# yukara-ikemiya/friendly-stable-audio-tools

Hardware: AMD Instinct MI355X
Metric: audio-seconds/sec @44.1kHz stereo, 100-step DPM++, SA-Open-1.0 shape (higher is better)
Workload: dtype fp16; 1 GPU; Stable-Audio-Open-1.0 DiT shape (24 layers, D=1536, S=1025, CFG 7 -> 2 sequences/prompt) + Oobleck decode, 1 prompt(s)/GPU x 47.55 s, 100 DPM-Solver++(3M) SDE steps; prompts_per_gpu=1, codec_dtype=fp16, sampler_steps=100, layernorm=fused, cross_attention=fused, sample_size=2097152, parallelism=dp1 (rank-strided prompts, one all-gather)

## Files before the change

### friendly-stable-audio-tools_amd/csrc/gemm_bf16.hip

```cpp
#include <stdlib.h>

#include <type_traits>

#include "attn_core.h"
#include <algorithm>

#include "sat_common.h"

namespace {

template <int EPI, int MI, int NI, bool LNC = false, bool QKN = false>
__device__ __forceinline__ void gemm_epilogue(const GemmArgs& g, f32x16 (&acc)[MI][NI], const int mw, const int nw, const int half,
                                              const int l31, const float2* ln = nullptr, const float* lc1 = nullptr,
                                              const float* lc2 = nullptr) {
    const int M = g.M, N = g.N;
    (void)N;

    if constexpr (EPI == EPI_F32) {
        float* __restrict__ C = g.C;
        const int ldc = g.ldc;
        float bia[NI];
#pragma unroll
        for (int j = 0; j < NI; ++j) bia[j] = g.bias ? g.bias[nw + j * 32 + l31] : 0.f;
        const bool accum = g.accumulate != 0;
// ... 344 lines not shown
            const int m = mw + i * 32 + l31;
            const int mc = m < M ? m : M - 1;
            const int b = mc / S;
            const int s = mc - b * S;
            const int ob = (kind & 4) ? ((b * S) & 3) : 0;
            if constexpr (LNC) {
                const float2 st = ln[i * 32 + l31];
#pragma unroll
                for (int j = 0; j < 2; ++j)
#pragma unroll
                    for (int q = 0; q < 4; ++q) {
                        const f32x4 c1 = *reinterpret_cast<const f32x4*>(lc1 + j * 32 + q * 8 + 4 * half);
                        const f32x4 c2 = *reinterpret_cast<const f32x4*>(lc2 + j * 32 + q * 8 + 4 * half);
#pragma unroll
                        for (int e = 0; e < 4; ++e) acc[i][j][4 * q + e] = st.y * (acc[i][j][4 * q + e] - st.x * c1[e]) + c2[e];
                    }
            }
            if constexpr (QKN) {
                if (kind & 16) {
                    float ss = 0.f;
#pragma unroll
                    for (int j = 0; j < 2; ++j)
#pragma unroll
                        for (int r = 0; r < 16; ++r) ss += acc[i][j][r] * acc[i][j][r];
                    unsigned a = __float_as_uint(ss), b = a;
                    half_swap(a, b);
                    const float inv = rsqrtf(fmaxf(__uint_as_float(a) + __uint_as_float(b), 1e-24f));
#pragma unroll
                    for (int j = 0; j < 2; ++j)
#pragma unroll
                        for (int r = 0; r < 16; ++r) acc[i][j][r] *= inv;
                }
            }
            if (kind & 2) {
                if constexpr (!ROPE_PRE) {
                    rcs[i][0] = *reinterpret_cast<const f32x4*>(he.rope_cos + (size_t)s * 16 + 4 * half);
                    rcs[i][1] = *reinterpret_cast<const f32x4*>(he.rope_cos + (size_t)s * 16 + 8 + 4 * half);
                    rsn[i][0] = *reinterpret_cast<const f32x4*>(he.rope_sin + (size_t)s * 16 + 4 * half);
                    rsn[i][1] = *reinterpret_cast<const f32x4*>(he.rope_sin + (size_t)s * 16 + 8 + 4 * half);
                }
                const f32x4 cs0 = rcs[i][0], cs1 = rcs[i][1], sn0 = rsn[i][0], sn1 = rsn[i][1];
#pragma unroll
                for (int r = 0; r < 8; ++r) {
                    const float cs = (r < 4) ? cs0[r & 3] : cs1[r & 3];
                    const float sn = (r < 4) ? sn0[r & 3] : sn1[r & 3];
                    const float x1 = acc[i][0][r], x2 = acc[i][0][r + 8];
                    acc[i][0][r] = x1 * cs - x2 * sn;
                    acc[i][0][r + 8] = x2 * cs + x1 * sn;
                }
            }
            if (kind & 8) {
#pragma unroll
                for (int j = 0; j < 2; ++j)
#pragma unroll
                    for (int r = 0; r < 16; ++r) acc[i][j][r] *= he.qscale;
            }
            op_t* row = dst + ((size_t)(b * he.heads + head) * Spad + s + ob) * 64 + 8 * half;
#pragma unroll
            for (int j = 0; j < 2; ++j) {
                unsigned pk[8];
#pragma unroll
                for (int q = 0; q < 4; ++q) {
                    pk[2 * q] = pack_op2(acc[i][j][4 * q], acc[i][j][4 * q + 1]);
                    pk[2 * q + 1] = pack_op2(acc[i][j][4 * q + 2], acc[i][j][4 * q + 3]);
                }
                half_swap(pk[0], pk[2]);
                half_swap(pk[1], pk[3]);
                half_swap(pk[4], pk[6]);
                half_swap(pk[5], pk[7]);
                if (qfrag) {
#pragma unroll
                    for (int e = 0; e < 8; ++e) qfrag[j][e] = pk[e];
                    continue;
                }
                if (m < M) {
                    *reinterpret_cast<u32x4*>(row + j * 32) = u32x4{pk[0], pk[1], pk[2], pk[3]};
                    *reinterpret_cast<u32x4*>(row + j * 32 + 16) = u32x4{pk[4], pk[5], pk[6], pk[7]};
                }
            }
        }
    }
}

template <int MI, bool PRE = false>
__device__ __forceinline__ void gemm_epilogue_f32_staged(const GemmArgs& g, f32x16 (&acc)[MI][2], float* ep, const int mw, const int nw,
                                                         const int lane, const f32x4* pre = nullptr) {
    const int half = lane >> 5, l31 = lane & 31;
    const int M = g.M;
    const int prow = lane >> 4;
    const int c4 = (lane & 15) * 4;
    const bool accum = g.accumulate != 0;
    const f32x4 bia = g.bias ? *reinterpret_cast<const f32x4*>(g.bias + nw + c4) : f32x4{0.f, 0.f, 0.f, 0.f};
#pragma unroll
    for (int i = 0; i < MI; ++i) {
#pragma unroll
        for (int j = 0; j < 2; ++j)
#pragma unroll
            for (int r = 0; r < 16; ++r) ep[((r & 3) + 8 * (r >> 2) + 4 * half) * 64 + j * 32 + l31] = acc[i][j][r];
#pragma unroll
        for (int grp = 0; grp < 2; ++grp) {
            f32x4 old[4];
#pragma unroll
            for (int p4 = 0; p4 < 4; ++p4) {
                const int m = mw + i * 32 + (grp * 4 + p4) * 4 + prow;
                if constexpr (PRE) old[p4] = pre[grp * 4 + p4];
                else old[p4] = (accum && m < M) ? *reinterpret_cast<const f32x4*>(g.C + (size_t)m * g.ldc + nw + c4) : f32x4{0.f, 0.f, 0.f, 0.f};
            }
#pragma unroll
            for (int p4 = 0; p4 < 4; ++p4) {
                const int row = (grp * 4 + p4) * 4 + prow;
                const int m = mw + i * 32 + row;
                f32x4 v = *reinterpret_cast<const f32x4*>(ep + row * 64 + c4) + bia;
                if (m < M && g.gate) v *= *reinterpret_cast<const f32x4*>(g.gate + (size_t)(m / g.gate_rows) * g.gate_ld + nw + c4);
                v += old[p4];
                if (m < M) *reinterpret_cast<f32x4*>(g.C + (size_t)m * g.ldc + nw + c4) = v;
                if (g.xb) {
                    opx4 xr;
                    float sum = 0.f, sq = 0.f;
#pragma unroll
                    for (int e = 0; e < 4; ++e) {
                        xr[e] = f32_to_op(v[e]);
                        const float f = op_to_f32(xr[e]);
                        sum += f;
                        sq += f * f;
                    }
                    sum = row16_sum(sum);
                    sq = row16_sum(sq);
                    if (m < M) {
                        *reinterpret_cast<opx4*>(g.xb + (size_t)m * g.N + nw + c4) = xr;
                        if ((lane & 15) == 0)
                            *reinterpret_cast<float2*>(g.ln_part_out + ((size_t)m * (g.N >> 6) + (nw >> 6)) * 2) = make_float2(sum, sq);
                    }
                }
            }
        }
    }
}

template <int BM, int BN, int WM, int WN, int EPIX>
__global__ __launch_bounds__(WM * WN * 64) void gemm_kernel(GemmArgs g) {
    sat_f16_saturate();
    constexpr int EPI = EPIX == EPI_HEADS_QKN ? EPI_HEADS : EPIX == EPI_ACT16 ? EPI_SWIGLU : EPIX;
    constexpr bool QKN = EPIX == EPI_HEADS_QKN || EPIX == EPI_ACT16;
    constexpr int NT = WM * WN * 64;
    constexpr int TM = BM / WM;
    constexpr int TN = BN / WN;
    static_assert(TN == 64, "wave tile is TM x 64");
    constexpr int MI = TM / 32;
    constexpr int NI = 2;
    constexpr int A_CH = BM * 8 / NT;
    constexpr int B_CH = BN * 8 / NT;
    static_assert(A_CH >= 1 && B_CH >= 1, "tile too small for the block");
    constexpr int STAGE_BYTES = (BM + BN) * 128;

    extern __shared__ __attribute__((aligned(16))) char smem[];

    const int tid = threadIdx.x;
    const int lane = tid & 63;
    const int wave = tid >> 6;
    const int wm = wave / WN;
    const int wn = wave % WN;
    const int half = lane >> 5;
    const int l31 = lane & 31;

    const int M = g.M, N = g.N, K = g.K;
    const int tiles_m = (M + BM - 1) / BM;
    const int tiles_n = N / BN;
    const int bid = xcd_remap(blockIdx.x, gridDim.x);
    int tm, tn;
    if (tiles_m <= tiles_n) {
        tn = bid / tiles_m;
        tm = bid - tn * tiles_m;
    } else {
        tm = bid / tiles_n;
        tn = bid - tm * tiles_n;
    }
    const int m0 = tm * BM;
    const int n0 = tn * BN;

    const op_t* __restrict__ A = g.A;
    const op_t* __restrict__ W = g.W;
// ... 110 lines not shown
    int tm, tn;
    if (tiles_m <= tiles_n) {
        tn = bid / tiles_m;
        tm = bid - tn * tiles_m;
    } else {
        tm = bid / tiles_n;
        tn = bid - tm * tiles_n;
    }
    const int m0 = tm * BM;
    const int n0 = tn * BN;

    const op_t* a_ptr[A_CH];
#pragma unroll
    for (int i = 0; i < A_CH; ++i) {
        int q = i * NT + tid;
        int row = q >> 3, pos = q & 7;
        int c = pos ^ ((row >> 1) & 7);
        int gm = m0 + row;
        gm = gm < M ? gm : M - 1;
        a_ptr[i] = g.A + (size_t)gm * K + c * 8;
    }
    const op_t* b_ptr[B_CH];
#pragma unroll
    for (int i = 0; i < B_CH; ++i) {
        int q = i * NT + tid;
        int row = q >> 3, pos = q & 7;
        int c = pos ^ ((row >> 1) & 7);
        b_ptr[i] = g.W + (size_t)(n0 + row) * K + c * 8;
    }

    f32x16 acc[MI][NI];
#pragma unroll
    for (int i = 0; i < MI; ++i)
#pragma unroll
        for (int j = 0; j < NI; ++j)
#pragma unroll
            for (int r = 0; r < 16; ++r) acc[i][j][r] = 0.f;

    auto stage_in = [&](int kt, int stage) {
        char* sa = smem + stage * STAGE_BYTES;
        char* sb = sa + BM * 128;
#pragma unroll
        for (int i = 0; i < A_CH; ++i)
            __builtin_amdgcn_global_load_lds((const __attribute__((address_space(1))) void*)(a_ptr[i] + kt * 64),
                                             (__attribute__((address_space(3))) void*)(sa + (i * NT + wave * 64) * 16), 16, 0, 0);
#pragma unroll
        for (int i = 0; i < B_CH; ++i)
            __builtin_amdgcn_global_load_lds((const __attribute__((address_space(1))) void*)(b_ptr[i] + kt * 64),
                                             (__attribute__((address_space(3))) void*)(sb + (i * NT + wave * 64) * 16), 16, 0, 0);
    };
    auto compute = [&](int stage) {
        const char* sa = smem + stage * STAGE_BYTES;
        const char* sb = sa + BM * 128;
#pragma unroll
        for (int ks = 0; ks < 4; ++ks) {
            opx8 af[MI], bfr[NI];
#pragma unroll
            for (int i = 0; i < MI; ++i)
                af[i] = *reinterpret_cast<const opx8*>(sa + lds_tile_off(wm * TM + i * 32 + l31, ks * 2 + half));
#pragma unroll
            for (int j = 0; j < NI; ++j)
                bfr[j] = *reinterpret_cast<const opx8*>(sb + lds_tile_off(wn * TN + j * 32 + l31, ks * 2 + half));
#pragma unroll
            for (int i = 0; i < MI; ++i)
#pragma unroll
                for (int j = 0; j < NI; ++j)
                    acc[i][j] = mfma_32x32x16(af[i], bfr[j], acc[i][j]);
        }
    };

    const int nk = K / 64;
    stage_in(0, 0);
    __syncthreads();
    for (int kt = 0; kt < nk - 1; ++kt) {
        stage_in(kt + 1, (kt + 1) & 1);
        compute(kt & 1);
        __syncthreads();
    }
    compute((nk - 1) & 1);

    gemm_epilogue<EPI, MI, NI, false, QKN>(g, acc, m0 + wm * TM, n0 + wn * TN, half, l31);
}

template <int BK>
__device__ __forceinline__ int lds_off_bk(int row, int chunk) {
    if constexpr (BK == 128) return row * 256 + ((chunk ^ (row & 15)) << 4);
    else if constexpr (BK == 64) return row * 128 + ((chunk ^ ((row >> 1) & 7)) << 4);
    else return row * 64 + ((chunk ^ ((row >> 2) & 3)) << 4);
}

template <int BM, int BN, int BK, int WM, int WN, int NS, int EPIX, int FP8 = 0, int KG = 1, bool DIL = false>
__global__ __launch_bounds__(KG * WM * WN * 64) void gemm_pipe_kernel(GemmArgs g) {
    sat_f16_saturate();
    constexpr int EPI = EPIX == EPI_HEADS_QKN ? EPI_HEADS : EPIX == EPI_ACT16 ? EPI_SWIGLU : EPIX;
    constexpr bool QKN = EPIX == EPI_HEADS_QKN || EPIX == EPI_ACT16;
    static_assert(!QKN || FP8 == 0, "qk_norm / plain activation: 16-bit operands only");
    static_assert(KG == 1 || (KG == 2 && EPI == EPI_F32 && FP8 == 0 && BK == 64 && BM / WM == 64 && BN / WN == 64),
                  "K-groups: fp32 output, 64 x 64 wave tiles, 128-byte rows");
    constexpr int NT = KG * WM * WN * 64;
    constexpr int TM = BM / WM;
    constexpr int TN = BN / WN;
    static_assert(TN == 64, "wave tile is TM x 64");
    constexpr int MI = TM / 32;
    constexpr int NI = TN / 32;
    constexpr int CPR = BK / 8;
    constexpr int NW = KG * WM * WN;
    constexpr int WL_A = BM * CPR / 64;
    constexpr int WLG = (BM + BN) * CPR / 64;
    constexpr int WL = KG * WLG;
    constexpr int LPT = (WL + NW - 1) / NW;
    constexpr int N_FULL = WL - (LPT - 1) * NW;
    constexpr bool UNIFORM = (WL % NW) == 0;
    constexpr int ROWB = BK * 2;
    constexpr bool MXA = FP8 == 3;
    constexpr int SCALE_WAVES = MXA ? BM / 64 : 0;
    constexpr int GROUP_BYTES = (BM + BN) * ROWB + (MXA ? BM * 4 : 0);
    constexpr int STAGE_BYTES = KG * GROUP_BYTES;
    constexpr int D = NS - 1;
    constexpr bool DIL_ON = (DIL || KG == 2) && FP8 == 0;
    constexpr int NDIL = !DIL_ON ? 0 : UNIFORM ? LPT : LPT - 1;
    constexpr int DIL_STEPS = KG == 2 ? BK / 32 : BK / 16 - 1;
    constexpr int DIL_PER = (NDIL + DIL_STEPS - 1) / (DIL_STEPS > 0 ? DIL_STEPS : 1);
    static_assert(!MXA || D == 1 || UNIFORM, "MXFP8: counted waits are built for uniform tiles or 2-stage rings");
    static_assert((BM * CPR) % 64 == 0 && (BN * CPR) % 64 == 0 && (D - 1) * LPT < 64, "bad pipeline geometry");
    static_assert(!FP8 || BK == 64, "fp8: 128-byte rows only");

    extern __shared__ __attribute__((aligned(16))) char smem[];

    const int tid = threadIdx.x;
    const int lane = tid & 63;
    const int wave = __builtin_amdgcn_readfirstlane(tid >> 6);
    const int grp = KG == 2 ? wave / (WM * WN) : 0;
    const int wv = KG == 2 ? wave % (WM * WN) : wave;
    const int wm = wv / WN;
    const int wn = wv % WN;
    const int half = lane >> 5;
    const int l31 = lane & 31;

    const int M = g.M, N = g.N, K = g.K;
    const int tiles_m = (M + BM - 1) / BM;
    const int tiles_n = N / BN;
    const int bid = xcd_remap(blockIdx.x, gridDim.x);
    int tm, tn;
    if (tiles_m <= tiles_n) {
        tn = bid / tiles_m;
        tm = bid - tn * tiles_m;
    } else {
        tm = bid / tiles_n;
        tn = bid - tm * tiles_n;
    }
    const int m0 = tm * BM;
    const int n0 = tn * BN;
    const bool wave_rows_valid = (m0 + wm * TM) < M;
    constexpr bool XA_OK = EPI == EPI_HEADS && MI == 1 && NI == 2 && NW == 4 && BN == 64 && BK == 64 && NS == 3 && FP8 == 0;
    constexpr int XA_OFF = (NS * STAGE_BYTES + (BM + BN) * 8 + 1023) & ~1023;
    [[maybe_unused]] bool xa_on = false;
    [[maybe_unused]] auto xa_stage = [&](int b) {
        const HeadsEpi& he = g.heads;
        const int kvh = (n0 >> 6) / (he.heads / he.xa_kvh);
        const op_t* kbase = he.xa_k + (size_t)(b * he.xa_kvh + kvh) * he.xa_sk_pad * 64;
        const op_t* vbase = he.xa_vt + (size_t)(b * he.xa_kvh + kvh) * 64 * he.xa_sk_pad;
        const int n_t = (((b * he.xa_sk) & 3) + he.xa_sk + 63) >> 6;
        for (int t = 0; t < n_t; ++t)
#pragma unroll
            for (int i = 0; i < 2; ++i) {
                const int p = wave + 4 * i;
                const int row = p * 8 + (lane >> 3);
                const int c = (lane & 7) ^ ((row >> 1) & 7);
                char* dst = smem + XA_OFF + t * 16384 + p * 1024;
                __builtin_amdgcn_global_load_lds((const __attribute__((address_space(1))) void*)(kbase + (size_t)(t * 64 + row) * 64 + c * 8),
                                                 (__attribute__((address_space(3))) void*)dst, 16, 0, 0);
                __builtin_amdgcn_global_load_lds((const __attribute__((address_space(1))) void*)(vbase + (size_t)row * he.xa_sk_pad + t * 64 + c * 8),
                                                 (__attribute__((address_space(3))) void*)(dst + 8192), 16, 0, 0);
            }
    };
    if constexpr (XA_OK) {
        xa_on = g.heads.xa_k != nullptr;
        if (xa_on) xa_stage(m0 / g.heads.S);
    }
    constexpr bool PRE_RESID = EPI == EPI_F32 && (MI == 1 || KG == 2) && NI == 2 && NT <= 512;
    const int epi_m = m0 + wm * TM + (KG == 2 ? grp * 32 : 0);
    const bool epi_rows_valid = KG == 2 ? epi_m < M : wave_rows_valid;
    [[maybe_unused]] f32x4 resid[PRE_RESID ? 8 : 1];
    if constexpr (PRE_RESID) {
        const bool want = g.accumulate != 0 && epi_rows_valid;
#pragma unroll
        for (int ps = 0; ps < 8; ++ps) {
            const int m = epi_m + ps * 4 + (lane >> 4);
            resid[ps] = (want && m < M) ? *reinterpret_cast<const f32x4*>(g.C + (size_t)m * g.ldc + n0 + wn * TN + (lane & 15) * 4)
                                        : f32x4{0.f, 0.f, 0.f, 0.f};
        }
    }

    constexpr bool LN_CONS = (EPI == EPI_SWIGLU || EPI == EPI_HEADS) && FP8 == 0;
    [[maybe_unused]] float2* lnst = reinterpret_cast<float2*>(smem + NS * STAGE_BYTES);
    [[maybe_unused]] float* lnc = reinterpret_cast<float*>(smem + NS * STAGE_BYTES + BM * 8);
    const op_t* ld_ptr[LPT];
#pragma unroll
    for (int i = 0; i < LPT; ++i) {
        const int L = KG == 2 ? grp * WLG + i * (WM * WN) + wv : i * NW + wave;
        const int lg = KG == 2 ? grp : 0;
        const int Lg = KG == 2 ? i * (WM * WN) + wv : L;
        const bool is_a = Lg < WL_A;
        int q = (is_a ? Lg : Lg - WL_A) * 64 + lane;
        int row = q / CPR, pos = q % CPR;
        int c = (BK == 128) ? (pos ^ (row & 15)) : (BK == 64) ? (pos ^ ((row >> 1) & 7)) : (pos ^ ((row >> 2) & 3));
        int gm = m0 + row;
        gm = gm < M ? gm : M - 1;
        int gn = n0 + row;
        gn = gn < N ? gn : N - 1;
        ld_ptr[i] = (is_a ? g.A + (size_t)gm * K + c * 8 : g.W + (size_t)gn * K + c * 8) + lg * BK;
    }
    const bool wave_full = UNIFORM || wave < N_FULL;
    [[maybe_unused]] const unsigned* sc_ptr = nullptr;
    if constexpr (MXA) {
        int gm = m0 + wave * 64 + lane;
        gm = gm < M ? gm : M - 1;
        sc_ptr = g.a_bscale + (size_t)gm * (K / BK);
    }

    f32x16 acc[MI][NI];
#pragma unroll
    for (int i = 0; i < MI; ++i)
#pragma unroll
        for (int j = 0; j < NI; ++j)
#pragma unroll
            for (int r = 0; r < 16; ++r) acc[i][j][r] = 0.f;
    auto stage_in = [&](int kt, int stage) {
        char* sa = smem + stage * STAGE_BYTES;
#pragma unroll
        for (int i = 0; i < LPT; ++i)
            if (UNIFORM || i + 1 < LPT || wave_full)
                __builtin_amdgcn_global_load_lds((const __attribute__((address_space(1))) void*)(ld_ptr[i] + kt * (BK * KG)),
                                                 (__attribute__((address_space(3))) void*)(sa + (KG == 2 ? grp * WLG + i * (WM * WN) + wv : i * NW + wave) * 1024), 16, 0, 0);
        if constexpr (MXA) {
            if (wave < SCALE_WAVES)
                __builtin_amdgcn_global_load_lds((const __attribute__((address_space(1))) void*)(sc_ptr + kt),
                                                 (__attribute__((address_space(3))) void*)(sa + (BM + BN) * ROWB + wave * 256), 4, 0, 0);
        }
    };
    [[maybe_unused]] auto wait_steady = [&]() {
        if constexpr (MXA && D > 1) {
            if (wave < SCALE_WAVES) wait_vmcnt<(D - 1) * (LPT + 1)>();
            else wait_vmcnt<(D - 1) * LPT>();
        } else if constexpr (UNIFORM || D == 1) {
            wait_vmcnt<(D - 1) * LPT>();
        } else {
            if (wave_full) wait_vmcnt<(D - 1) * LPT>();
            else wait_vmcnt<(D - 1) * (LPT - 1)>();
        }
    };
    typedef long i64x2 __attribute__((ext_vector_type(2)));
    auto compute = [&](int stage, auto trc, [[maybe_unused]] int kt_issue = -1, [[maybe_unused]] int st_issue = 0) {
        constexpr bool TRc = decltype(trc)::value;
        const char* sa = smem + stage * STAGE_BYTES + grp * GROUP_BYTES;
        const char* sb = sa + BM * ROWB;
        constexpr int KS = BK / 16;
        if constexpr (FP8 >= 2) {
            typedef int i32x8 __attribute__((ext_vector_type(8)));
            constexpr int KS2 = BK / 32;
            i32x8 af[2][MI], bfr[2][NI];
            auto frag = [&](int ks, int buf) {
#pragma unroll
                for (int i = 0; i < MI; ++i) {
                    const int row = wm * TM + i * 32 + l31;
                    u32x4 lo = *reinterpret_cast<const u32x4*>(sa + lds_off_bk<BK>(row, ks * 4 + half));
                    u32x4 hi = *reinterpret_cast<const u32x4*>(sa + lds_off_bk<BK>(row, ks * 4 + 2 + half));
                    af[buf][i] = i32x8{(int)lo[0], (int)lo[1], (int)lo[2], (int)lo[3], (int)hi[0], (int)hi[1], (int)hi[2], (int)hi[3]};
                }
#pragma unroll
                for (int j = 0; j < NI; ++j) {
                    const int row = wn * TN + j * 32 + l31;
                    u32x4 lo = *reinterpret_cast<const u32x4*>(sb + lds_off_bk<BK>(row, ks * 4 + half));
                    u32x4 hi = *reinterpret_cast<const u32x4*>(sb + lds_off_bk<BK>(row, ks * 4 + 2 + half));
                    bfr[buf][j] = i32x8{(int)lo[0], (int)lo[1], (int)lo[2], (int)lo[3], (int)hi[0], (int)hi[1], (int)hi[2], (int)hi[3]};
                }
            };
            constexpr bool DBUF = NT < 1024;
            [[maybe_unused]] int sdw[MI];
            if constexpr (MXA) {
                const char* ssc = sb + BN * ROWB;
#pragma unroll
                for (int i = 0; i < MI; ++i)
                    sdw[i] = (int)(*reinterpret_cast<const unsigned*>(ssc + (wm * TM + i * 32 + l31) * 4) >> (8 * half));
            }
            auto mx = [&](const i32x8& af_, const i32x8& bf_, f32x16 c_, int ks, int i) -> f32x16 {
                if constexpr (MXA) {
                    static_assert(!TRc, "MXFP8 A operand: block scales were probed on the A side only (tools/mx_probe.cpp)");
                    if (ks == 0) return __builtin_amdgcn_mfma_scale_f32_32x32x64_f8f6f4(af_, bf_, c_, 0, 0, 0, sdw[i], 0, 0x7F7F7F7F);
                    return __builtin_amdgcn_mfma_scale_f32_32x32x64_f8f6f4(af_, bf_, c_, 0, 0, 2, sdw[i], 0, 0x7F7F7F7F);
                } else if constexpr (TRc) {
                    return __builtin_amdgcn_mfma_scale_f32_32x32x64_f8f6f4(bf_, af_, c_, 0, 0, 0, 0x7F7F7F7F, 0, 0x7F7F7F7F);
                } else {
                    return __builtin_amdgcn_mfma_scale_f32_32x32x64_f8f6f4(af_, bf_, c_, 0, 0, 0, 0x7F7F7F7F, 0, 0x7F7F7F7F);
                }
            };
            if constexpr (!DBUF) {
#pragma unroll
                for (int ks = 0; ks < KS2; ++ks) {
                    frag(ks, 0);
#pragma unroll
                    for (int i = 0; i < MI; ++i)
#pragma unroll
                        for (int j = 0; j < NI; ++j)
                            acc[i][j] = mx(af[0][i], bfr[0][j], acc[i][j], ks, i);
                }
                return;
            }
            frag(0, 0);
            __builtin_amdgcn_sched_group_barrier(0x100, 2 * (MI + NI), 0);
#pragma unroll
            for (int ks = 0; ks < KS2; ++ks) {
                if (ks + 1 < KS2) frag(ks + 1, (ks + 1) & 1);
#pragma unroll
                for (int i = 0; i < MI; ++i)
#pragma unroll
                    for (int j = 0; j < NI; ++j)
                        acc[i][j] = mx(af[ks & 1][i], bfr[ks & 1][j], acc[i][j], ks, i);
                if (ks + 1 < KS2) {
                    constexpr int NR = 2 * (MI + NI), NM = MI * NI;
#pragma unroll
                    for (int r = 0; r < NM; ++r) {
                        __builtin_amdgcn_sched_group_barrier(0x8, 1, 0);
                        __builtin_amdgcn_sched_group_barrier(0x100, NR / NM, 0);
                    }
                    if (NR % NM) __builtin_amdgcn_sched_group_barrier(0x100, NR % NM, 0);
                } else {
                    __builtin_amdgcn_sched_group_barrier(0x8, MI * NI, 0);
                }
            }
            return;
        }
        if constexpr (FP8 == 1) {
            i64x2 af[2][MI], bfr[2][NI];
            auto frag = [&](int ks, int buf) {
#pragma unroll
                for (int i = 0; i < MI; ++i)
                    af[buf][i] = *reinterpret_cast<const i64x2*>(sa + lds_off_bk<BK>(wm * TM + i * 32 + l31, ks * 2 + half));
#pragma unroll
                for (int j = 0; j < NI; ++j)
                    bfr[buf][j] = *reinterpret_cast<const i64x2*>(sb + lds_off_bk<BK>(wn * TN + j * 32 + l31, ks * 2 + half));
            };
            frag(0, 0);
            __builtin_amdgcn_sched_group_barrier(0x100, MI + NI, 0);
#pragma unroll
            for (int ks = 0; ks < KS; ++ks) {
                if (ks + 1 < KS) frag(ks + 1, (ks + 1) & 1);
#pragma unroll
                for (int h2 = 0; h2 < 2; ++h2)
#pragma unroll
                    for (int i = 0; i < MI; ++i)
#pragma unroll
                        for (int j = 0; j < NI; ++j)
                            acc[i][j] = TRc ? __builtin_amdgcn_mfma_f32_32x32x16_fp8_fp8(bfr[ks & 1][j][h2], af[ks & 1][i][h2], acc[i][j], 0, 0, 0)
                                            : __builtin_amdgcn_mfma_f32_32x32x16_fp8_fp8(af[ks & 1][i][h2], bfr[ks & 1][j][h2], acc[i][j], 0, 0, 0);
                if (ks + 1 < KS) {
#pragma unroll
                    for (int r = 0; r < MI + NI; ++r) {
                        __builtin_amdgcn_sched_group_barrier(0x8, 1, 0);
                        __builtin_amdgcn_sched_group_barrier(0x100, 1, 0);
                    }
                    __builtin_amdgcn_sched_group_barrier(0x8, 2 * MI * NI - (MI + NI), 0);
                } else {
                    __builtin_amdgcn_sched_group_barrier(0x8, 2 * MI * NI, 0);
                }
            }
            return;
        }
        opx8 af[2][MI], bfr[2][NI];
        auto frag = [&](int ks, int buf) {
#pragma unroll
            for (int i = 0; i < MI; ++i)
                af[buf][i] = *reinterpret_cast<const opx8*>(sa + lds_off_bk<BK>(wm * TM + i * 32 + l31, ks * 2 + half));
#pragma unroll
            for (int j = 0; j < NI; ++j)
                bfr[buf][j] = *reinterpret_cast<const opx8*>(sb + lds_off_bk<BK>(wn * TN + j * 32 + l31, ks * 2 + half));
        };
        frag(0, 0);
        __builtin_amdgcn_sched_group_barrier(0x100, MI + NI, 0);
#pragma unroll
        for (int ks = 0; ks < KS; ++ks) {
            if (ks + 1 < KS) frag(ks + 1, (ks + 1) & 1);
            if constexpr (DIL_ON) {
                if (ks < DIL_STEPS && kt_issue >= 0) {
                    char* sdst = smem + st_issue * STAGE_BYTES;
#pragma unroll
                    for (int i = ks * DIL_PER; i < (ks + 1) * DIL_PER && i < NDIL; ++i)
                        __builtin_amdgcn_global_load_lds((const __attribute__((address_space(1))) void*)(ld_ptr[i] + kt_issue * (BK * KG)),
                                                         (__attribute__((address_space(3))) void*)(sdst + (KG == 2 ? grp * WLG + i * (WM * WN) + wv : i * NW + wave) * 1024), 16, 0, 0);
                }
            }
#pragma unroll
            for (int i = 0; i < MI; ++i)
#pragma unroll
                for (int j = 0; j < NI; ++j)
                    acc[i][j] = TRc ? mfma_32x32x16(bfr[ks & 1][j], af[ks & 1][i], acc[i][j])
                                    : mfma_32x32x16(af[ks & 1][i], bfr[ks & 1][j], acc[i][j]);
            if (ks + 1 < KS) {
                constexpr int NR = MI + NI, NM = MI * NI;
                if constexpr (KG == 2) {
                    __builtin_amdgcn_sched_group_barrier(0x8, 1, 0);
                    __builtin_amdgcn_sched_group_barrier(0x100, NR, 0);
                    if (ks < KS / 2 && DIL_PER == 4) {
                        __builtin_amdgcn_sched_group_barrier(0x8, 1, 0);
                        __builtin_amdgcn_sched_group_barrier(0x20, 2, 0);
                        __builtin_amdgcn_sched_group_barrier(0x8, 1, 0);
                        __builtin_amdgcn_sched_group_barrier(0x20, 2, 0);
                        __builtin_amdgcn_sched_group_barrier(0x8, 1, 0);
                    } else {
                        __builtin_amdgcn_sched_group_barrier(0x8, NM - 1, 0);
                    }
                } else {
#pragma unroll
                    for (int r = 0; r < (NR < NM ? NR : NM); ++r) {
                        __builtin_amdgcn_sched_group_barrier(0x8, 1, 0);
                        __builtin_amdgcn_sched_group_barrier(0x100, 1, 0);
                    }
                    if (NM > NR) __builtin_amdgcn_sched_group_barrier(0x8, NM - NR, 0);
                    if (NR > NM) __builtin_amdgcn_sched_group_barrier(0x100, NR - NM, 0);
                    if (DIL_ON && ks < DIL_STEPS) __builtin_amdgcn_sched_group_barrier(0x20, DIL_PER, 0);
                }
            } else {
                __builtin_amdgcn_sched_group_barrier(0x8, MI * NI, 0);
            }
            if constexpr (KG == 2) {
                if (ks == KS / 2 - 1) {
                    __builtin_amdgcn_sched_barrier(0);
                    __builtin_amdgcn_s_barrier();
                    __builtin_amdgcn_sched_barrier(0);
                }
            }
        }
    };

    const int nk = K / (BK * KG);
#pragma unroll
    for (int s = 0; s < D; ++s) stage_in(s, s);
    if constexpr (LN_CONS) {
        const bool ln_fold = g.ln_part != nullptr;
        constexpr int TPR = (NT / BM >= 4) ? 4 : (NT / BM >= 2 ? 2 : 1);
        const int np = K >> 6;
        const int r = tid / TPR, sub = tid % TPR;
        float sum = 0.f, sq = 0.f;
        if (ln_fold && r < BM) {
            int m = m0 + r;
            m = m < M ? m : M - 1;
            const float2* pp = reinterpret_cast<const float2*>(g.ln_part) + (size_t)m * np;
// ... 97 lines not shown
            const int m = m0 + wm * TM + l31;
            const int b_me = (m < M ? m : M - 1) / S;
            const int last = (m0 + BM - 1 < M ? m0 + BM - 1 : M - 1);
            const int b_lo = m0 / S, b_hi = last / S;
            const int wlast = (m0 + wm * TM + 31 < M ? m0 + wm * TM + 31 : M - 1);
            const int w_lo = (m0 + wm * TM) / S, w_hi = wlast / S;
            for (int bb = b_lo; bb <= b_hi; ++bb) {
                if (bb > b_lo) {
                    __builtin_amdgcn_s_barrier();
                    xa_stage(bb);
                    wait_vmcnt<0>();
                    __builtin_amdgcn_s_barrier();
                }
                if (!(wave_rows_valid && w_lo <= bb && bb <= w_hi)) continue;
                const int ob = (bb * he.xa_sk) & 3, k_end = ob + he.xa_sk;
                const int n_t = (k_end + 63) >> 6;
                attn::State<2> st;
                st.init(half);
                for (int t = 0; t < n_t; ++t) {
                    const char* sk = smem + XA_OFF + t * 16384;
                    const bool edge = (t == 0 && ob != 0) || (t == n_t - 1 && (k_end & 63) != 0);
                    attn::tile<2>(st, qf, sk, sk + 8192, edge, t * 64, ob, k_end, t == 0, 1.0f, l31, half);
                }
                const float inv = 1.0f / attn::half_sum(st.l_run);
                op_t* op = he.xa_out + (size_t)m * ((size_t)he.heads * 64) + n0 + 8 * half;
#pragma unroll
                for (int db = 0; db < 2; ++db) {
                    unsigned pk[8];
#pragma unroll
                    for (int rq = 0; rq < 4; ++rq) {
                        pk[2 * rq] = pack_op2(st.oacc[db][rq * 4] * inv, st.oacc[db][rq * 4 + 1] * inv);
                        pk[2 * rq + 1] = pack_op2(st.oacc[db][rq * 4 + 2] * inv, st.oacc[db][rq * 4 + 3] * inv);
                    }
                    half_swap(pk[0], pk[2]);
                    half_swap(pk[1], pk[3]);
                    half_swap(pk[4], pk[6]);
                    half_swap(pk[5], pk[7]);
                    if (m < M && b_me == bb) {
                        *reinterpret_cast<u32x4*>(op + db * 32) = u32x4{pk[0], pk[1], pk[2], pk[3]};
                        *reinterpret_cast<u32x4*>(op + db * 32 + 16) = u32x4{pk[4], pk[5], pk[6], pk[7]};
                    }
                }
            }
            return;
        }
    }
    if constexpr (FP8 != 0) {
        __builtin_amdgcn_sched_barrier(0);
        if (wave_rows_valid) {
            if (tr) {
#pragma unroll
                for (int i = 0; i < MI; ++i) {
                    int row = m0 + wm * TM + i * 32 + l31;
                    row = row < M ? row : M - 1;
                    const float sa_r = g.a_scale[row];
#pragma unroll
                    for (int j = 0; j < NI; ++j)
#pragma unroll
                        for (int q = 0; q < 4; ++q) {
                            const f32x4 sw = *reinterpret_cast<const f32x4*>(g.w_scale + n0 + wn * TN + j * 32 + q * 8 + 4 * half);
#pragma unroll
                            for (int e = 0; e < 4; ++e) acc[i][j][4 * q + e] *= sa_r * sw[e];
                        }
                }
            } else {
                float sw[NI];
#pragma unroll
                for (int j = 0; j < NI; ++j) sw[j] = g.w_scale[n0 + wn * TN + j * 32 + l31];
#pragma unroll
                for (int i = 0; i < MI; ++i)
#pragma unroll
                    for (int r = 0; r < 16; ++r) {
                        int row = m0 + wm * TM + i * 32 + (r & 3) + 8 * (r >> 2) + 4 * half;
                        row = row < M ? row : M - 1;
                        const float sa_r = MXA ? 1.0f : g.a_scale[row];
#pragma unroll
                        for (int j = 0; j < NI; ++j) acc[i][j][r] *= sa_r * sw[j];
                    }
            }
        }
    }
    if constexpr (KG == 2) {
        __builtin_amdgcn_s_barrier();
        float* mine = reinterpret_cast<float*>(smem) + wave * 2048;
#pragma unroll
        for (int j = 0; j < 2; ++j)
#pragma unroll
            for (int r = 0; r < 16; ++r) mine[(j * 16 + r) * 64 + lane] = grp ? acc[0][j][r] : acc[1][j][r];
        __syncthreads();
        const float* theirs = reinterpret_cast<const float*>(smem) + (wave ^ (WM * WN)) * 2048;
        f32x16 fin[1][2];
#pragma unroll
        for (int j = 0; j < 2; ++j)
#pragma unroll
            for (int r = 0; r < 16; ++r) fin[0][j][r] = (grp ? acc[1][j][r] : acc[0][j][r]) + theirs[(j * 16 + r) * 64 + lane];
        static_assert(KG == 1 || NS * STAGE_BYTES >= 2 * NW * 8192, "exchange + staging areas");
        if (epi_rows_valid)
            gemm_epilogue_f32_staged<1, true>(g, fin, reinterpret_cast<float*>(smem + NW * 8192) + wave * 2048, epi_m, n0 + wn * TN, lane, resid);
        return;
    }
    if constexpr (EPI == EPI_F32) {
        __builtin_amdgcn_s_barrier();
        if (wave_rows_valid) {
            if constexpr (PRE_RESID)
                gemm_epilogue_f32_staged<MI, true>(g, acc, reinterpret_cast<float*>(smem) + wave * 2048, m0 + wm * TM, n0 + wn * TN, lane, resid);
            else
                gemm_epilogue_f32_staged<MI>(g, acc, reinterpret_cast<float*>(smem) + wave * 2048, m0 + wm * TM, n0 + wn * TN, lane);
        }
    } else if (wave_rows_valid) {
        if (tr) gemm_epilogue_t<EPI, MI, NI, LN_CONS, (NT < 1024), QKN>(g, acc, m0 + wm * TM, n0 + wn * TN, half, l31, lnst + wm * TM, lnc + wn * TN, lnc + BN + wn * TN);
        else gemm_epilogue<EPI, MI, NI, LN_CONS, QKN>(g, acc, m0 + wm * TM, n0 + wn * TN, half, l31, lnst + wm * TM, lnc + wn * TN, lnc + BN + wn * TN);
    }
}

template <int BM, int BN, int BK, int WM, int WN, int NS, int EPIX, int FP8 = 0, int KG = 1, bool DIL = false>
int launch_pipe(const GemmArgs& a, hipStream_t stream) {
    constexpr int EPI = EPIX == EPI_HEADS_QKN ? EPI_HEADS : EPIX == EPI_ACT16 ? EPI_SWIGLU : EPIX;
    constexpr int NT = KG * WM * WN * 64;
    constexpr bool LN_CONS = (EPI == EPI_SWIGLU || EPI == EPI_HEADS) && FP8 == 0;
    constexpr int LDS = NS * KG * ((BM + BN) * BK * 2 + (FP8 == 3 ? BM * 4 : 0)) + (LN_CONS ? (BM + BN) * 8 : 0);
    static_assert(LDS <= 160 * 1024, "LDS ring exceeds 160 KiB");
    SAT_CHECK_ARG(LN_CONS || !a.ln_part, SAT_E_UNSUPPORTED, "gemm: LayerNorm fold needs bf16 operands and a SwiGLU / heads epilogue");
    SAT_CHECK_ARG((!a.xb && !a.ln_part_out) || (EPI == EPI_F32 && BN / WN == 64 && FP8 == 0 && a.xb && a.ln_part_out), SAT_E_UNSUPPORTED,
                  "gemm: the bf16 image / row statistics come from the bf16 fp32-output tiles with 64-column wave tiles");
    static_assert(EPI != EPI_F32 || BN / WN != 64 || LDS >= WM * WN * 8192, "the staged fp32 epilogue needs 8 KiB of LDS per wave");
    auto kern = gemm_pipe_kernel<BM, BN, BK, WM, WN, NS, EPIX, FP8, KG, DIL>;
    constexpr bool XA_OK = EPI == EPI_HEADS && BM == 128 && BN == 64 && BK == 64 && WM == 4 && WN == 1 && NS == 3 && FP8 == 0;
    constexpr int XA_LDS = XA_OK ? ((NS * (BM + BN) * BK * 2 + (BM + BN) * 8 + 1023) & ~1023) + 3 * 16384 : LDS;
    static_assert(XA_LDS <= 160 * 1024, "fused cross-attention: K / V^T tiles do not fit behind the ring");
    bool xa = false;
    if constexpr (EPI == EPI_HEADS) {
        xa = a.heads.xa_k != nullptr;
        if (xa) {
            const HeadsEpi& he = a.heads;
            SAT_CHECK_ARG(XA_OK, SAT_E_UNSUPPORTED, "gemm: the fused cross-attention epilogue lives in the 128 x 64 tile (variant 16)");
            SAT_CHECK_ARG(he.parts == 1 && (he.kind[0] & ~16) == 8 && he.qscale == SAT_ATTN_QSCALE && he.xa_vt && he.xa_out && he.xa_kvh > 0 &&
                              he.heads % he.xa_kvh == 0 && he.xa_sk > 0 && he.xa_sk + 3 <= 192 && he.xa_sk_pad >= he.xa_sk + 3 && he.xa_sk_pad % 64 == 0,
                          SAT_E_UNSUPPORTED, "gemm: fused cross-attention needs one pre-scaled row-major part and at most 189 keys (got %d)", he.xa_sk);
        }
    }
    SAT_TRY(sat_ensure_dynamic_lds(reinterpret_cast<const void*>(kern), XA_LDS));
    GemmArgs b = a;
    if (FP8) {
        SAT_CHECK_ARG(a.K % 128 == 0 && a.w_scale && (FP8 == 3 ? (const void*)a.a_bscale : (const void*)a.a_scale), SAT_E_UNSUPPORTED,
                      "gemm(fp8): K=%d must be a multiple of 128 and both scale vectors given", a.K);
        b.K = a.K / 2;
    }
    SAT_CHECK_ARG(b.N % BN == 0, SAT_E_UNSUPPORTED, "gemm: N=%d not a multiple of the %d-column tile", b.N, BN);
    SAT_CHECK_ARG(b.K % (BK * KG) == 0 && b.K / (BK * KG) >= NS, SAT_E_UNSUPPORTED, "gemm: K=%d too small for the %d-stage pipeline", a.K, NS);
    int tiles = cdiv(b.M, BM) * (b.N / BN);
    hipLaunchKernelGGL(kern, dim3(tiles), dim3(NT), xa ? XA_LDS : LDS, stream, b);
    SAT_LAUNCH_CHECK();
    return 0;
}

template <int BM, int BN, int WM, int WN, int EPI, bool GLDS = false>
int launch_cfg(const GemmArgs& a, hipStream_t stream) {
    constexpr int NT = WM * WN * 64;
    constexpr int LDS = 2 * (BM + BN) * 128;
    SAT_CHECK_ARG(!a.ln_part && !a.xb && !a.ln_part_out, SAT_E_UNSUPPORTED, "gemm: LayerNorm fold is built into the pipelined tiles only (K >= 192)");
    auto kern = GLDS ? gemm_glds_kernel<BM, BN, WM, WN, EPI> : gemm_kernel<BM, BN, WM, WN, EPI>;
    SAT_TRY(sat_ensure_dynamic_lds(reinterpret_cast<const void*>(kern), LDS));
    SAT_CHECK_ARG(a.N % BN == 0, SAT_E_UNSUPPORTED, "gemm: N=%d not a multiple of the %d-column tile", a.N, BN);
    int tiles = cdiv(a.M, BM) * (a.N / BN);
    hipLaunchKernelGGL(kern, dim3(tiles), dim3(NT), LDS, stream, a);
    SAT_LAUNCH_CHECK();
    return 0;
}

template <int ID, int EPI, int F8>
int launch_tile(const GemmArgs& a, hipStream_t stream) {
    constexpr SatTile t = sat_tile_geom(ID);
    static_assert(!t.f32_only || EPI == EPI_F32, "tile built for the fp32-output epilogue only");
    if constexpr (t.family == SAT_GEMM_PIPE) return launch_pipe<t.bm, t.bn, t.bk, t.wm, t.wn, t.ns, EPI, F8, t.kg, t.dil && F8 == 0>(a, stream);
    else return launch_cfg<t.bm, t.bn, t.wm, t.wn, EPI, t.family == SAT_GEMM_DMA2>(a, stream);
}

template <int EPI, int F8>
int launch_epi(int tile, const GemmArgs& a, hipStream_t stream) {
#define SAT_TILE_CASE(id) \
    case id: return launch_tile<id, EPI, F8>(a, stream);
    switch (tile) {
        SAT_TILE_CASE(SAT_TILE_128)
        SAT_TILE_CASE(SAT_TILE_128x64)
        SAT_TILE_CASE(SAT_TILE_256)
        SAT_TILE_CASE(SAT_TILE_256x192)
    }
// ... 101 lines not shown
```

Measured before the change: 76.24 audio-seconds/sec.

## Use 16x16x32 MFMA fragments for fp32-output pipelined GEMMs with 512 threads

```diff
diff --git a/friendly-stable-audio-tools_amd/csrc/gemm_bf16.hip b/friendly-stable-audio-tools_amd/csrc/gemm_bf16.hip
--- a/friendly-stable-audio-tools_amd/csrc/gemm_bf16.hip
+++ b/friendly-stable-audio-tools_amd/csrc/gemm_bf16.hip
@@ -450,10 +450,28 @@
     }
 }
 
-template <int MI, bool PRE = false>
-__device__ __forceinline__ void gemm_epilogue_f32_staged(const GemmArgs& g, f32x16 (&acc)[MI][2], float* ep, const int mw, const int nw,
+template <int MI>
+__device__ __forceinline__ void stage_rows32(float* ep, const f32x16 (&acc)[MI][2], const int i, const int lane) {
+    const int half = lane >> 5, l31 = lane & 31;
+#pragma unroll
+    for (int j = 0; j < 2; ++j)
+#pragma unroll
+        for (int r = 0; r < 16; ++r) ep[((r & 3) + 8 * (r >> 2) + 4 * half) * 64 + j * 32 + l31] = acc[i][j][r];
+}
+template <int MB>
+__device__ __forceinline__ void stage_rows32(float* ep, const f32x4 (&acc)[MB][4], const int i, const int lane) {
+    const int l15 = lane & 15, q = lane >> 4;
+#pragma unroll
+    for (int rb = 0; rb < 2; ++rb)
+#pragma unroll
+        for (int cb = 0; cb < 4; ++cb)
+#pragma unroll
+            for (int r = 0; r < 4; ++r) ep[(rb * 16 + 4 * q + r) * 64 + cb * 16 + l15] = acc[2 * i + rb][cb][r];
+}
+
+template <int MI, bool PRE = false, typename Acc>
+__device__ __forceinline__ void gemm_epilogue_f32_staged(const GemmArgs& g, Acc& acc, float* ep, const int mw, const int nw,
                                                          const int lane, const f32x4* pre = nullptr) {
-    const int half = lane >> 5, l31 = lane & 31;
     const int M = g.M;
     const int prow = lane >> 4;
     const int c4 = (lane & 15) * 4;
@@ -461,10 +479,7 @@
     const f32x4 bia = g.bias ? *reinterpret_cast<const f32x4*>(g.bias + nw + c4) : f32x4{0.f, 0.f, 0.f, 0.f};
 #pragma unroll
     for (int i = 0; i < MI; ++i) {
-#pragma unroll
-        for (int j = 0; j < 2; ++j)
-#pragma unroll
-            for (int r = 0; r < 16; ++r) ep[((r & 3) + 8 * (r >> 2) + 4 * half) * 64 + j * 32 + l31] = acc[i][j][r];
+        stage_rows32(ep, acc, i, lane);
 #pragma unroll
         for (int grp = 0; grp < 2; ++grp) {
             f32x4 old[4];
@@ -741,6 +756,12 @@
     gemm_epilogue<EPI, MI, NI, false, QKN>(g, acc, m0 + wm * TM, n0 + wn * TN, half, l31);
 }
 
+#ifdef SAT_RING_MFMA_32X32
+constexpr bool SAT_RING_MFMA_16 = false;
+#else
+constexpr bool SAT_RING_MFMA_16 = true;
+#endif
+
 template <int BK>
 __device__ __forceinline__ int lds_off_bk(int row, int chunk) {
     if constexpr (BK == 128) return row * 256 + ((chunk ^ (row & 15)) << 4);
@@ -759,6 +780,8 @@
     constexpr int NT = KG * WM * WN * 64;
     constexpr int TM = BM / WM;
     constexpr int TN = BN / WN;
+    constexpr bool S16 = SAT_RING_MFMA_16 && EPI == EPI_F32 && FP8 == 0 && NT == 512;
+    static_assert(!S16 || BK == 64, "16 x 16 x 32 fragments: two 32-k steps per 128-byte row");
     static_assert(TN == 64, "wave tile is TM x 64");
     constexpr int MI = TM / 32;
     constexpr int NI = TN / 32;
@@ -778,7 +801,8 @@
     constexpr int D = NS - 1;
     constexpr bool DIL_ON = (DIL || KG == 2) && FP8 == 0;
     constexpr int NDIL = !DIL_ON ? 0 : UNIFORM ? LPT : LPT - 1;
-    constexpr int DIL_STEPS = KG == 2 ? BK / 32 : BK / 16 - 1;
+    constexpr int DIL_STEPS = KG == 2 ? (S16 ? 1 : BK / 32) : BK / 16 - 1;
+    static_assert(!S16 || KG == 2 || !DIL_ON, "16 x 16 x 32, one K-group: the LDS-DMA pieces are issued in front of compute()");
     constexpr int DIL_PER = (NDIL + DIL_STEPS - 1) / (DIL_STEPS > 0 ? DIL_STEPS : 1);
     static_assert(!MXA || D == 1 || UNIFORM, "MXFP8: counted waits are built for uniform tiles or 2-stage rings");
     static_assert((BM * CPR) % 64 == 0 && (BN * CPR) % 64 == 0 && (D - 1) * LPT < 64, "bad pipeline geometry");
@@ -885,6 +909,12 @@
         for (int j = 0; j < NI; ++j)
 #pragma unroll
             for (int r = 0; r < 16; ++r) acc[i][j][r] = 0.f;
+    constexpr int MB = S16 ? TM / 16 : 1;
+    [[maybe_unused]] f32x4 acc16[MB][4];
+#pragma unroll
+    for (int i = 0; i < MB; ++i)
+#pragma unroll
+        for (int j = 0; j < 4; ++j) acc16[i][j] = f32x4{0.f, 0.f, 0.f, 0.f};
     auto stage_in = [&](int kt, int stage) {
         char* sa = smem + stage * STAGE_BYTES;
 #pragma unroll
@@ -1022,6 +1052,77 @@
                     __builtin_amdgcn_sched_group_barrier(0x8, 2 * MI * NI - (MI + NI), 0);
                 } else {
                     __builtin_amdgcn_sched_group_barrier(0x8, 2 * MI * NI, 0);
+                }
+            }
+            return;
+        }
+        if constexpr (S16) {
+            static_assert(!TRc, "16 x 16 x 32: fp32 output, un-swapped");
+            constexpr int KS2 = BK / 32, NR = MB + 4, NM = MB * 4;
+            const int l15 = lane & 15, q = lane >> 4;
+            opx8 af[2][MB], bfr[2][4];
+            auto frag = [&](int ks, int buf) {
+#pragma unroll
+                for (int i = 0; i < MB; ++i)
+                    af[buf][i] = *reinterpret_cast<const opx8*>(sa + lds_off_bk<BK>(wm * TM + i * 16 + l15, ks * 4 + q));
+#pragma unroll
+                for (int j = 0; j < 4; ++j)
+                    bfr[buf][j] = *reinterpret_cast<const opx8*>(sb + lds_off_bk<BK>(wn * TN + j * 16 + l15, ks * 4 + q));
+            };
+            frag(0, 0);
+            __builtin_amdgcn_sched_group_barrier(0x100, NR, 0);
+#pragma unroll
+            for (int ks = 0; ks < KS2; ++ks) {
+                if (ks + 1 < KS2) frag(ks + 1, (ks + 1) & 1);
+                if constexpr (KG == 2) {
+                    if (ks < DIL_STEPS && kt_issue >= 0) {
+                        char* sdst = smem + st_issue * STAGE_BYTES;
+#pragma unroll
+                        for (int i = ks * DIL_PER; i < (ks + 1) * DIL_PER && i < NDIL; ++i)
+                            __builtin_amdgcn_global_load_lds((const __attribute__((address_space(1))) void*)(ld_ptr[i] + kt_issue * (BK * KG)),
+                                                             (__attribute__((address_space(3))) void*)(sdst + (grp * WLG + i * (WM * WN) + wv) * 1024), 16, 0, 0);
+                    }
+                }
+#pragma unroll
+                for (int i = 0; i < MB; ++i)
+#pragma unroll
+                    for (int j = 0; j < 4; ++j) acc16[i][j] = mfma_16x16x32(af[ks & 1][i], bfr[ks & 1][j], acc16[i][j]);
+                if constexpr (KG == 2) {
+                    if (ks + 1 < KS2) {
+                        __builtin_amdgcn_sched_group_barrier(0x8, 1, 0);
+                        __builtin_amdgcn_sched_group_barrier(0x100, NR / 2, 0);
+                        __builtin_amdgcn_sched_group_barrier(0x8, 1, 0);
+                        __builtin_amdgcn_sched_group_barrier(0x100, NR - NR / 2, 0);
+                        if (DIL_PER == 8 && NM == 16) {
+                            __builtin_amdgcn_sched_group_barrier(0x8, 1, 0);
+#pragma unroll
+                            for (int r = 0; r < 4; ++r) {
+                                __builtin_amdgcn_sched_group_barrier(0x8, 1, 0);
+                                __builtin_amdgcn_sched_group_barrier(0x20, 2, 0);
+                                __builtin_amdgcn_sched_group_barrier(0x8, 2, 0);
+                            }
+                            __builtin_amdgcn_sched_group_barrier(0x8, 1, 0);
+                        } else {
+                            __builtin_amdgcn_sched_group_barrier(0x8, NM - 2, 0);
+                        }
+                    } else {
+                        __builtin_amdgcn_sched_group_barrier(0x8, NM, 0);
+                    }
+                    if (ks == KS2 / 2 - 1) {
+                        __builtin_amdgcn_sched_barrier(0);
+                        __builtin_amdgcn_s_barrier();
+                        __builtin_amdgcn_sched_barrier(0);
+                    }
+                } else if (ks + 1 < KS2) {
+#pragma unroll
+                    for (int r = 0; r < (NR < NM ? NR : NM); ++r) {
+                        __builtin_amdgcn_sched_group_barrier(0x8, 1, 0);
+                        __builtin_amdgcn_sched_group_barrier(0x100, 1, 0);
+                    }
+                    if (NM > NR) __builtin_amdgcn_sched_group_barrier(0x8, NM - NR, 0);
+                    if (NR > NM) __builtin_amdgcn_sched_group_barrier(0x100, NR - NM, 0);
+                } else {
+                    __builtin_amdgcn_sched_group_barrier(0x8, NM, 0);
                 }
             }
             return;
@@ -1285,6 +1386,32 @@
     }
     if constexpr (KG == 2) {
         __builtin_amdgcn_s_barrier();
+        if constexpr (S16) {
+            f32x4* mine = reinterpret_cast<f32x4*>(smem) + wave * 512;
+#pragma unroll
+            for (int rb = 0; rb < 2; ++rb)
+#pragma unroll
+                for (int cb = 0; cb < 4; ++cb) {
+                    f32x4 v;
+#pragma unroll
+                    for (int e = 0; e < 4; ++e) v[e] = grp ? acc16[rb][cb][e] : acc16[2 + rb][cb][e];
+                    mine[(rb * 4 + cb) * 64 + lane] = v;
+                }
+            __syncthreads();
+            const f32x4* theirs = reinterpret_cast<const f32x4*>(smem) + (wave ^ (WM * WN)) * 512;
+            f32x4 fin[2][4];
+#pragma unroll
+            for (int rb = 0; rb < 2; ++rb)
+#pragma unroll
+                for (int cb = 0; cb < 4; ++cb) {
+                    const f32x4 t = theirs[(rb * 4 + cb) * 64 + lane];
+#pragma unroll
+                    for (int e = 0; e < 4; ++e) fin[rb][cb][e] = (grp ? acc16[2 + rb][cb][e] : acc16[rb][cb][e]) + t[e];
+                }
+            if (epi_rows_valid)
+                gemm_epilogue_f32_staged<1, true>(g, fin, reinterpret_cast<float*>(smem + NW * 8192) + wave * 2048, epi_m, n0 + wn * TN, lane, resid);
+            return;
+        }
         float* mine = reinterpret_cast<float*>(smem) + wave * 2048;
 #pragma unroll
         for (int j = 0; j < 2; ++j)
@@ -1305,7 +1432,11 @@
     if constexpr (EPI == EPI_F32) {
         __builtin_amdgcn_s_barrier();
         if (wave_rows_valid) {
-            if constexpr (PRE_RESID)
+            if constexpr (S16 && PRE_RESID)
+                gemm_epilogue_f32_staged<MI, true>(g, acc16, reinterpret_cast<float*>(smem) + wave * 2048, m0 + wm * TM, n0 + wn * TN, lane, resid);
+            else if constexpr (S16)
+                gemm_epilogue_f32_staged<MI>(g, acc16, reinterpret_cast<float*>(smem) + wave * 2048, m0 + wm * TM, n0 + wn * TN, lane);
+            else if constexpr (PRE_RESID)
                 gemm_epilogue_f32_staged<MI, true>(g, acc, reinterpret_cast<float*>(smem) + wave * 2048, m0 + wm * TM, n0 + wn * TN, lane, resid);
             else
                 gemm_epilogue_f32_staged<MI>(g, acc, reinterpret_cast<float*>(smem) + wave * 2048, m0 + wm * TM, n0 + wn * TN, lane);
```

New measurement: 77.30 audio-seconds/sec, median of 6. 1.4% higher.
